# wangjie212/ManiSDP-matlab

Measured on AMD Instinct MI355X. Metric: tCG Hess-vec prods/sec (n,p), G81 MaxCut, higher is better.
Workload: dtype f64; 1 GPU; Gset G81 MaxCut, ManiSDP_onlyunitdiag RTR call, n=20000, p=32; n=20000, p=32, nnz_C=92644, TR_maxiter=40, TR_maxinner=100, parallelism=rows1

## Files before the change

manisdp-matlab_amd/csrc/msdp_pipe.h:

```cpp
#pragma once
#include <type_traits>
#include "msdp_psync.h"

template <class F>
__device__ __forceinline__ bool psync8(unsigned long long* slots, unsigned gen, int G, double (&v)[8], double* sh8, double* shb8, int* err,
                                       int bid, int backoff, unsigned long long* tr, F on_ready) {
    const int lane = threadIdx.x & 63, w = threadIdx.x >> 6;
    {
        const bool h8 = (lane & 8) != 0;
        double a[4], b[2], x;
#pragma unroll
        for (int k = 0; k < 4; ++k) a[k] = msdp_swap_add<32>(v[k], v[4 + k]);
#pragma unroll
        for (int k = 0; k < 2; ++k) b[k] = msdp_swap_add<16>(a[k], a[2 + k]);
        x = (h8 ? b[1] : b[0]) + msdp_dpp<0x128>(h8 ? b[0] : b[1]);
        x += msdp_dpp<MSDP_DPP_XOR1>(x); x += msdp_dpp<MSDP_DPP_XOR2>(x); x += msdp_dpp<MSDP_DPP_HALF_MIRROR>(x);
        if ((lane & 7) == 0) sh8[(lane >> 3) * PWAVES + w] = x;
    }
    if (tr && threadIdx.x == 0) tr[4] = __builtin_readcyclecounter();
    asm volatile("s_waitcnt vmcnt(0)" ::: "memory");
    __syncthreads();
    if (tr && threadIdx.x == 0) tr[2] = __builtin_readcyclecounter();
    {
        unsigned long long* gbase = slots + (size_t)(gen % PSYNC_GEN) * PSYNC_REP * PSYNC_NV * MSDP_MAX_GRID;
        if (w == 0) {
            const int rep = lane / PSYNC_NV, vi = lane % PSYNC_NV;
            double s = 0.0;
            for (int i = 0; i < PWAVES; ++i) s += sh8[vi * PWAVES + i];
            asm volatile("s_waitcnt vmcnt(0)" ::: "memory");
            __hip_atomic_store(gbase + ((size_t)rep * PSYNC_NV + vi) * MSDP_MAX_GRID + bid,
                               (unsigned long long)__double_as_longlong(s), __ATOMIC_RELAXED, __HIP_MEMORY_SCOPE_AGENT);
        }
        const unsigned long long* p0 = gbase + ((size_t)(bid & (PSYNC_REP - 1)) * PSYNC_NV + w) * MSDP_MAX_GRID + lane;
        double r0;
        int spins = 0;
        bool fail = false;
        const int first = ((backoff >> 16) & 0xff) ? ((backoff >> 16) & 0xff) : 27;
        for (int q = 0; q < first; ++q) __builtin_amdgcn_s_sleep(1);
        if (tr && threadIdx.x == 0) tr[3] = __builtin_readcyclecounter();
        for (;;) {
            unsigned long long b0[4];
            asm volatile(
                "global_load_dwordx2 %0, %4, off sc1\n\t"
                "global_load_dwordx2 %1, %4, off offset:512 sc1\n\t"
                "global_load_dwordx2 %2, %4, off offset:1024 sc1\n\t"
                "global_load_dwordx2 %3, %4, off offset:1536 sc1\n\t"
                "s_waitcnt vmcnt(0)"
                : "=&v"(b0[0]), "=&v"(b0[1]), "=&v"(b0[2]), "=&v"(b0[3])
                : "v"(p0)
                : "memory");
            bool ok = true;
            double t0 = 0.0;
#pragma unroll
            for (int q = 0; q < 4; ++q) {
                if (lane + 64 * q < G) {
                    ok = ok && b0[q] != PSYNC_SENT;
                    t0 += __longlong_as_double((long long)b0[q]);
                }
            }
            r0 = t0;
            if (__builtin_amdgcn_ballot_w64(!ok) == 0ULL) break;
            ++spins;
            if (spins > PSYNC_SPIN_LIMIT ||
                ((spins & 1023) == 0 && __hip_atomic_load(err, __ATOMIC_RELAXED, __HIP_MEMORY_SCOPE_AGENT))) { fail = true; break; }
            for (int q = 0; q < ((backoff >> 8) & 0xff); ++q) __builtin_amdgcn_s_sleep(1);
        }
        if (tr && threadIdx.x == 0) tr[7] = (__builtin_readcyclecounter() << 4) + (unsigned long long)(spins < 15 ? spins : 15);
        if (!fail) on_ready();
        r0 = msdp_wave_sum(r0);
        if (lane == 0) {
            shb8[w] = r0; shb8[8 + w] = fail ? 1.0 : 0.0;
            if (fail) __hip_atomic_store(err, 1, __ATOMIC_RELAXED, __HIP_MEMORY_SCOPE_AGENT);
        }
        if (w == 0)
            __hip_atomic_store(slots + (size_t)((gen + PSYNC_GEN - 1) % PSYNC_GEN) * PSYNC_REP * PSYNC_NV * MSDP_MAX_GRID +
                                   (size_t)lane * MSDP_MAX_GRID + bid,
                               PSYNC_SENT, __ATOMIC_RELAXED, __HIP_MEMORY_SCOPE_AGENT);
    }
    asm volatile("s_waitcnt lgkmcnt(0)\n\ts_barrier" ::: "memory");
    double bad = 0.0;
#pragma unroll
    for (int i = 0; i < 8; ++i) { v[i] = msdp_readlane(shb8[i], 0); bad += msdp_readlane(shb8[8 + i], 0); }
    return bad == 0.0;
}

typedef unsigned long long v2ul __attribute__((ext_vector_type(2)));
template <class F>
__device__ __forceinline__ bool psync8_lines(unsigned long long* slots, unsigned gen, int G, double (&v)[8], double* sh8, double* shp, double* shb8,
                                             int* err, int bid, int backoff, unsigned long long* tr, F on_ready) {
    const int lane = threadIdx.x & 63, w = threadIdx.x >> 6;
    {
        const bool h8 = (lane & 8) != 0;
        double a[4], b[2], x;
#pragma unroll
        for (int k = 0; k < 4; ++k) a[k] = msdp_swap_add<32>(v[k], v[4 + k]);
#pragma unroll
        for (int k = 0; k < 2; ++k) b[k] = msdp_swap_add<16>(a[k], a[2 + k]);
        x = (h8 ? b[1] : b[0]) + msdp_dpp_all<0x128>(h8 ? b[0] : b[1]);
        x += msdp_dpp_all<MSDP_DPP_XOR1>(x); x += msdp_dpp_all<MSDP_DPP_XOR2>(x); x += msdp_dpp_all<MSDP_DPP_HALF_MIRROR>(x);
        if ((lane & 7) == 0) sh8[(lane >> 3) * PWAVES + w] = x;
    }
    if (tr && threadIdx.x == 0) tr[4] = __builtin_readcyclecounter();
    asm volatile("s_waitcnt vmcnt(0)" ::: "memory");
    __syncthreads();
    if (tr && threadIdx.x == 0) tr[2] = __builtin_readcyclecounter();
    unsigned long long* gbase = slots + (size_t)(gen % PSYNC_GEN) * PSYNC_REP * PSYNC_NV * MSDP_MAX_GRID;
    if (w == 0) {
        const int rep = lane >> 3, vi = lane & 7;
        double s = 0.0;
        for (int i = 0; i < PWAVES; ++i) s += sh8[vi * PWAVES + i];
        asm volatile("s_waitcnt vmcnt(0)" ::: "memory");
        __hip_atomic_store(gbase + (size_t)rep * PSYNC_NV * MSDP_MAX_GRID + (size_t)bid * 8 + vi,
                           (unsigned long long)__double_as_longlong(s), __ATOMIC_RELAXED, __HIP_MEMORY_SCOPE_AGENT);
    }
    const unsigned long long* p0 = gbase + (size_t)(bid & (PSYNC_REP - 1)) * PSYNC_NV * MSDP_MAX_GRID + (size_t)(32 * w + (lane >> 2)) * 8 + 2 * (lane & 3);
    const bool in0 = 32 * w + (lane >> 2) < G, in1 = 32 * w + 16 + (lane >> 2) < G;
    double t0 = 0.0, t1 = 0.0;
    int spins = 0;
    bool fail = false;
    const int first = ((backoff >> 16) & 0xff) ? ((backoff >> 16) & 0xff) : (backoff & 0xff);
    for (int q = 0; q < first; ++q) __builtin_amdgcn_s_sleep(1);
    if (tr && threadIdx.x == 0) tr[3] = __builtin_readcyclecounter();
    if (__builtin_amdgcn_ballot_w64(in0) != 0ULL) {
        for (;;) {
            v2ul a0, a1;
            asm volatile(
                "global_load_dwordx4 %0, %2, off sc1\n\t"
                "global_load_dwordx4 %1, %2, off offset:1024 sc1\n\t"
                "s_waitcnt vmcnt(0)"
                : "=&v"(a0), "=&v"(a1)
                : "v"(p0)
                : "memory");
            bool ok = true;
            t0 = 0.0; t1 = 0.0;
            if (in0) { ok = a0.x != PSYNC_SENT && a0.y != PSYNC_SENT; t0 = __longlong_as_double((long long)a0.x); t1 = __longlong_as_double((long long)a0.y); }
            if (in1) { ok = ok && a1.x != PSYNC_SENT && a1.y != PSYNC_SENT; t0 += __longlong_as_double((long long)a1.x); t1 += __longlong_as_double((long long)a1.y); }
            if (__builtin_amdgcn_ballot_w64(!ok) == 0ULL) break;
            ++spins;
            if (spins > PSYNC_SPIN_LIMIT ||
                ((spins & 1023) == 0 && __hip_atomic_load(err, __ATOMIC_RELAXED, __HIP_MEMORY_SCOPE_AGENT))) { fail = true; break; }
            for (int q = 0; q < ((backoff >> 8) & 0xff); ++q) __builtin_amdgcn_s_sleep(1);
        }
    }
    if (tr && threadIdx.x == 0) tr[7] = (__builtin_readcyclecounter() << 4) + (unsigned long long)(spins < 15 ? spins : 15);
    t0 += msdp_dpp_all<0x124>(t0); t1 += msdp_dpp_all<0x124>(t1);
    t0 += msdp_dpp_all<0x128>(t0); t1 += msdp_dpp_all<0x128>(t1);
    t0 = msdp_rowpair_sum<16>(t0); t1 = msdp_rowpair_sum<16>(t1);
    t0 = msdp_rowpair_sum<32>(t0); t1 = msdp_rowpair_sum<32>(t1);
    if (lane < 4) { shp[w * 8 + 2 * lane] = t0; shp[w * 8 + 2 * lane + 1] = t1; }
    if (lane == 0) {
        shb8[8 + w] = fail ? 1.0 : 0.0;
        if (fail) __hip_atomic_store(err, 1, __ATOMIC_RELAXED, __HIP_MEMORY_SCOPE_AGENT);
    }
    asm volatile("s_waitcnt lgkmcnt(0)\n\ts_barrier" ::: "memory");
    on_ready();
    if (w == 0)
        __hip_atomic_store(slots + (size_t)((gen + PSYNC_GEN - 1) % PSYNC_GEN) * PSYNC_REP * PSYNC_NV * MSDP_MAX_GRID +
                               (size_t)(lane >> 3) * PSYNC_NV * MSDP_MAX_GRID + (size_t)bid * 8 + (lane & 7),
                           PSYNC_SENT, __ATOMIC_RELAXED, __HIP_MEMORY_SCOPE_AGENT);
    double s = 0.0;
#pragma unroll
    for (int k = 0; k < PWAVES; ++k) s += shp[k * 8 + (lane & 7)];
    const double fl = shb8[8 + (lane & 7)];
#pragma unroll
    for (int i = 0; i < 8; ++i) v[i] = msdp_readlane(s, i);
    return __builtin_amdgcn_ballot_w64(fl != 0.0) == 0ULL;
}

__device__ __forceinline__ bool pbar8_lines(unsigned long long* slots, unsigned gen, int G, double* shb8, int* err, int bid, int backoff) {
    const int lane = threadIdx.x & 63, w = threadIdx.x >> 6;
    asm volatile("s_waitcnt vmcnt(0)" ::: "memory");
    __syncthreads();
    unsigned long long* gbase = slots + (size_t)(gen % PSYNC_GEN) * PSYNC_REP * PSYNC_NV * MSDP_MAX_GRID;
    if (w == 0) {
        asm volatile("s_waitcnt vmcnt(0)" ::: "memory");
        __hip_atomic_store(gbase + (size_t)(lane >> 3) * PSYNC_NV * MSDP_MAX_GRID + (size_t)bid * 8 + (lane & 7), 0ULL, __ATOMIC_RELAXED, __HIP_MEMORY_SCOPE_AGENT);
    }
    const unsigned long long* p0 = gbase + (size_t)(bid & (PSYNC_REP - 1)) * PSYNC_NV * MSDP_MAX_GRID + (size_t)(32 * w + (lane >> 2)) * 8 + 2 * (lane & 3);
    const bool in0 = 32 * w + (lane >> 2) < G, in1 = 32 * w + 16 + (lane >> 2) < G;
    int spins = 0;
    bool fail = false;
    const int first = ((backoff >> 16) & 0xff) ? ((backoff >> 16) & 0xff) : (backoff & 0xff);
    for (int q = 0; q < first; ++q) __builtin_amdgcn_s_sleep(1);
    if (__builtin_amdgcn_ballot_w64(in0) != 0ULL) {
        for (;;) {
            v2ul a0, a1;
            asm volatile(
                "global_load_dwordx4 %0, %2, off sc1\n\t"
                "global_load_dwordx4 %1, %2, off offset:1024 sc1\n\t"
                "s_waitcnt vmcnt(0)"
                : "=&v"(a0), "=&v"(a1)
                : "v"(p0)
                : "memory");
            bool ok = true;
            if (in0) ok = a0.x != PSYNC_SENT && a0.y != PSYNC_SENT;
            if (in1) ok = ok && a1.x != PSYNC_SENT && a1.y != PSYNC_SENT;
            if (__builtin_amdgcn_ballot_w64(!ok) == 0ULL) break;
            ++spins;
            if (spins > PSYNC_SPIN_LIMIT ||
                ((spins & 1023) == 0 && __hip_atomic_load(err, __ATOMIC_RELAXED, __HIP_MEMORY_SCOPE_AGENT))) { fail = true; break; }
            for (int q = 0; q < ((backoff >> 8) & 0xff); ++q) __builtin_amdgcn_s_sleep(1);
        }
    }
    if (lane == 0) {
        shb8[8 + w] = fail ? 1.0 : 0.0;
        if (fail) __hip_atomic_store(err, 1, __ATOMIC_RELAXED, __HIP_MEMORY_SCOPE_AGENT);
    }
    asm volatile("s_waitcnt lgkmcnt(0)\n\ts_barrier" ::: "memory");
    if (w == 0)
        __hip_atomic_store(slots + (size_t)((gen + PSYNC_GEN - 1) % PSYNC_GEN) * PSYNC_REP * PSYNC_NV * MSDP_MAX_GRID +
                               (size_t)(lane >> 3) * PSYNC_NV * MSDP_MAX_GRID + (size_t)bid * 8 + (lane & 7),
                           PSYNC_SENT, __ATOMIC_RELAXED, __HIP_MEMORY_SCOPE_AGENT);
    const double fl = shb8[8 + (lane & 7)];
    return __builtin_amdgcn_ballot_w64(fl != 0.0) == 0ULL;
}

template <class F>
__device__ __forceinline__ bool psync2_8(unsigned long long* blk, unsigned long long* const* peers, int N, int me, int ri, unsigned gen, int G,
                                         double (&v)[8], double* sh8, double* shb8, int* err, int bid, int backoff, F on_ready) {
    const int lane = threadIdx.x & 63, w = threadIdx.x >> 6;
    {
        const bool h8 = (lane & 8) != 0;
        double a[4], b[2], x;
#pragma unroll
        for (int k = 0; k < 4; ++k) a[k] = msdp_swap_add<32>(v[k], v[4 + k]);
#pragma unroll
        for (int k = 0; k < 2; ++k) b[k] = msdp_swap_add<16>(a[k], a[2 + k]);
        x = (h8 ? b[1] : b[0]) + msdp_dpp<0x128>(h8 ? b[0] : b[1]);
        x += msdp_dpp<MSDP_DPP_XOR1>(x); x += msdp_dpp<MSDP_DPP_XOR2>(x); x += msdp_dpp<MSDP_DPP_HALF_MIRROR>(x);
        if ((lane & 7) == 0) sh8[(lane >> 3) * PWAVES + w] = x;
    }
    asm volatile("s_waitcnt vmcnt(0)" ::: "memory");
    __syncthreads();
    unsigned long long* ls = blk + (size_t)ri * XR2_REGION;
    unsigned long long* ml = ls + PSYNC_REGION;
    unsigned long long* gbase = ls + (size_t)(gen % PSYNC_GEN) * PSYNC_REP * PSYNC_NV * MSDP_MAX_GRID;
    if (w == 0 && lane < 8) {
        double s = 0.0;
        for (int i = 0; i < PWAVES; ++i) s += sh8[lane * PWAVES + i];
        asm volatile("s_waitcnt vmcnt(0)" ::: "memory");
        __hip_atomic_store(gbase + (size_t)lane * MSDP_MAX_GRID + bid, (unsigned long long)__double_as_longlong(s), __ATOMIC_RELAXED, __HIP_MEMORY_SCOPE_AGENT);
    }
    bool fail = false;
    if (bid == 0) {
        const unsigned long long* p0 = gbase + (size_t)w * MSDP_MAX_GRID + lane;
        double r0 = 0.0;
        int spins = 0;
        for (;;) {
            unsigned long long b0[4];
            asm volatile(
                "global_load_dwordx2 %0, %4, off sc1\n\t"
                "global_load_dwordx2 %1, %4, off offset:512 sc1\n\t"
                "global_load_dwordx2 %2, %4, off offset:1024 sc1\n\t"
                "global_load_dwordx2 %3, %4, off offset:1536 sc1\n\t"
                "s_waitcnt vmcnt(0)"
                : "=&v"(b0[0]), "=&v"(b0[1]), "=&v"(b0[2]), "=&v"(b0[3])
                : "v"(p0)
                : "memory");
            bool ok = true;
            double t0 = 0.0;
#pragma unroll
            for (int q = 0; q < 4; ++q) {
                if (lane + 64 * q < G) {
                    ok = ok && b0[q] != PSYNC_SENT;
                    t0 += __longlong_as_double((long long)b0[q]);
                }
            }
            r0 = t0;
            if (__builtin_amdgcn_ballot_w64(!ok) == 0ULL) break;
            ++spins;
            if (spins > PSYNC_SPIN_LIMIT || ((spins & 1023) == 0 && __hip_atomic_load(err, __ATOMIC_RELAXED, __HIP_MEMORY_SCOPE_AGENT))) { fail = true; break; }
        }
        r0 = msdp_wave_sum(r0);
        if (!fail && lane < N)
            __hip_atomic_store(peers[lane] + (size_t)ri * XR2_REGION + PSYNC_REGION + ((size_t)(gen % PSYNC_GEN) * 8 + me) * 8 + w,
                               (unsigned long long)__double_as_longlong(r0), __ATOMIC_RELAXED, __HIP_MEMORY_SCOPE_SYSTEM);
        if (fail) xr2_fail(blk, peers, N, err);
        if (w > 0 && lane == 0) shb8[8 + w] = fail ? 1.0 : 0.0;
    }
    if (w == 0) {
        const unsigned long long* p = ml + (size_t)(gen % PSYNC_GEN) * 64 + lane;
        const bool need = (lane >> 3) < N;
        const int first = bid == 0 ? 0 : (((backoff >> 16) & 0xff) ? ((backoff >> 16) & 0xff) : (backoff & 0xff));
        for (int q = 0; q < first; ++q) __builtin_amdgcn_s_sleep(1);
        unsigned long long x = 0ULL;
        int spins = 0;
        for (;;) {
            x = ld_u64_sys(p);
            if (__builtin_amdgcn_ballot_w64(need && x == PSYNC_SENT) == 0ULL) break;
            ++spins;
            if (spins > PSYNC_SPIN_LIMIT || ((spins & 1023) == 0 && __hip_atomic_load(err, __ATOMIC_RELAXED, __HIP_MEMORY_SCOPE_AGENT))) { fail = true; break; }
            for (int q = 0; q < ((backoff >> 8) & 0xff); ++q) __builtin_amdgcn_s_sleep(1);
        }
        double t = need ? __longlong_as_double((long long)x) : 0.0;
        t += msdp_dpp<0x128>(t);
        t = msdp_rowpair_sum<16>(t);
        t = msdp_rowpair_sum<32>(t);
        if (lane < 8) { shb8[lane] = t; if (bid != 0 && lane > 0) shb8[8 + lane] = 0.0; }
        if (lane == 0) shb8[8] = fail ? 1.0 : 0.0;
        if (fail) xr2_fail(blk, peers, N, err);
        if (lane < PSYNC_NV)
            __hip_atomic_store(ls + (size_t)((gen + PSYNC_GEN - 1) % PSYNC_GEN) * PSYNC_REP * PSYNC_NV * MSDP_MAX_GRID + (size_t)lane * MSDP_MAX_GRID + bid,
                               PSYNC_SENT, __ATOMIC_RELAXED, __HIP_MEMORY_SCOPE_AGENT);
        if (bid == 0)
            __hip_atomic_store(ml + (size_t)((gen + PSYNC_GEN - 1) % PSYNC_GEN) * 64 + lane, PSYNC_SENT, __ATOMIC_RELAXED, __HIP_MEMORY_SCOPE_AGENT);
    }
    __syncthreads();
    on_ready();
    double bad = 0.0;
#pragma unroll
    for (int i = 0; i < 8; ++i) { v[i] = msdp_readlane(shb8[i], 0); bad += msdp_readlane(shb8[8 + i], 0); }
    return bad == 0.0;
}

#ifndef MSDP_PIPE_LINES
#define MSDP_PIPE_LINES 1
#endif
#if MSDP_PIPE_LINES
#define PSYNC8(slots, gen, G, v, sh8, shb8, err, bid, backoff, tr, f) psync8_lines(slots, gen, G, v, sh8, shp, shb8, err, bid, backoff, tr, f)
#else
#define PSYNC8(slots, gen, G, v, sh8, shb8, err, bid, backoff, tr, f) psync8(slots, gen, G, v, sh8, shb8, err, bid, backoff, tr, f)
#endif
template <int LPR, int EW, int R, bool TRACE, bool FUSE, int XRM = 0, int EP = 1>
__device__ __forceinline__ void tcg_pipe_body(const Dev& d, unsigned long long* slots, int* err, const int bx) {
    constexpr bool XR = XRM != 0, XTWO = XRM == 2;
    constexpr bool CSR = EW == 0;
    static_assert(!XR || (!FUSE && !TRACE), "cross-rank instances: per-iteration launches");
    static_assert(R <= 5, "pipelined trip: every vector in registers");
    static_assert(CSR ? (EP == 64 / LPR && !XR && !TRACE) : EP == 1, "CSR rows: one row per wave, one rank");
    static_assert(PSYNC_NV == 8 && PSYNC_REP * PSYNC_NV == 64, "psync8 posts one slot per lane of wave 0");
    constexpr bool BSTORE = XRM == 0 && EW == 5 && !(FUSE && LPR == 8);
    constexpr bool BOFF = !(EW == 8 && LPR == 16), ROWB_INV = !XTWO;
    extern __shared__ double lds[];
    __shared__ double sh8[8 * PWAVES];
    __shared__ double shp[8 * PWAVES];
    __shared__ double shb8[16];
    constexpr int RPW = 64 / (LPR * EP);
    constexpr int RSTEP = PWAVES * RPW;
    constexpr int ROWS = R * RSTEP;
    double2* Ys = reinterpret_cast<double2*>(lds);
    double2* Gs = Ys + R * PB;
    double* eGs = reinterpret_cast<double*>(Gs + R * PB);
    double* vs = eGs + ROWS;
    int* cs = reinterpret_cast<int*>(vs + EW * ROWS);
    int* ls = cs + EW * ROWS;
    double2* HQs = reinterpret_cast<double2*>(ls + EW * ROWS);
    unsigned long long* pds = reinterpret_cast<unsigned long long*>(HQs + 2 * R * PB);
    double2* YPs = HQs + 2 * R * PB;
    double2* GPs = YPs + R * PB;
    double* EGPs = reinterpret_cast<double*>(GPs + R * PB);

    const Ctl* c = d.ctl;
    const bool lead = bx == 0 && threadIdx.x == 0;
    const int k_tr = c->k;
    if (c->done) {
        if (lead) {
            frame_store(&d.F[0], c->gg, c->gg, 0.0, 0.0, 0.0, sqrt(c->gg), 0.0, 0.0, 0, 0, 5, 0, 0, 1);
            d.ctl->tcg_running = 0;
            msdp_publish(d, k_tr, 0, 0);
        }
        return;
    }
    if (lead && !FUSE) msdp_publish(d, k_tr, 0, 1);
    const int bid = (XR && !XTWO) ? d.xr_gid0 + bx : bx;
    const int GS = (XR && !XTWO) ? d.xr_gtot : d.G;
    const int xri = k_tr & 1;
    __shared__ unsigned long long* shpeer[XTWO ? 8 : 1];
    if (XTWO) {
        if (threadIdx.x < 8) shpeer[threadIdx.x] = threadIdx.x < d.xr2_n ? d.xr2_peers[threadIdx.x] : d.xr2_blk;
        psync2_reset_other(d.xr2_blk, xri ^ 1, bid, GS);
        asm volatile("s_waitcnt vmcnt(0)" ::: "memory");
    } else if (XR) {
        unsigned long long* other = slots + (size_t)(xri ^ 1) * PSYNC_REGION;
        slots += (size_t)xri * PSYNC_REGION;
        psync_reset_other(other, bid, GS);
        asm volatile("s_waitcnt vmcnt(0)" ::: "memory");
    } else if (!FUSE) psync_reset_other(slots + PSYNC_REGION, bid, GS);
    int lo, hi;
    msdp_chunk_rows(d.n_loc, d.G, lo, hi, 0, bx);
    const int lane = threadIdx.x & 63, wave = threadIdx.x >> 6;
    const int sub = lane & (LPR - 1), rsub = lane / (LPR * EP);
    const int epi = (lane / LPR) & (EP - 1);
    const bool colok_g = 2 * sub < d.ld;
    const bool colok = colok_g && epi == 0;
    int cur = c->cur;
    const bool bench = c->bench_mode != 0;
    double Delta = c->Delta;
    const double kappa = c->kappa, theta = c->theta;
    const int mininner = c->mininner, maxinner = c->maxinner;
    double gg = c->gg;
    double fx = c->fx;
    int k_it = c->k;
    const double Delta_bar = c->Delta_bar, rho_prime = c->rho_prime, rho_reg_opt = c->rho_reg, tolgradnorm = c->tolgradnorm;
    const int maxiter = c->maxiter;
    int n_acc = c->accepted, n_rej = c->rejected, n_hv = c->hessvecs, n_ce = c->cost_evals;
    const double* __restrict__ Yl = cur ? d.Y[1] : d.Y[0];
    const double* __restrict__ gl = cur ? d.Gr[1] : d.Gr[0];
    const double* __restrict__ eGl = cur ? d.eG[1] : d.eG[0];
    const int slot0 = wave * RPW + rsub;
#define SLOT(r) ((r) * RSTEP + slot0)
#define ROW(r) (lo + SLOT(r))
#define ROK(r) (ROW(r) < hi)
#define OK(r) (ROK(r) && colok)
    const unsigned rowb0 = ((unsigned)(lo + slot0) * (unsigned)d.ld + 2u * (unsigned)sub) * 8u;
#define ROWB(r) (ROWB_INV ? (rowb0 + (unsigned)((r) * RSTEP) * (unsigned)d.ld * 8u) : (((unsigned)ROW(r) * gld + 2 * sub) * 8u))
    const int refresh = c->pipe_refresh;
    const int backoff = (c->psync_backoff & 0xff00ffff) | ((((c->psync_backoff >> 16) & 0xff) ? ((c->psync_backoff >> 16) & 0xff) : (c->psync8_backoff & 0xff)) << 16);
    const double2 zz = make_double2(0.0, 0.0);
    const unsigned gld = (unsigned)d.ld;
    constexpr bool LOC = !CSR && R * EW <= 15;
    constexpr bool MULTI = LOC && !(FUSE && LPR >= 16);
    double2 eta[R], rr[R], md[R], hmd[R], cmd[R], ctr[R];
#pragma unroll
    for (int r = 0; r < R; ++r) {
        const bool rok = ROK(r);
        const int rc = rok ? ROW(r) : lo;
        const int64_t o = (int64_t)rc * d.ld + (colok ? 2 * sub : 0);
        double2 y = ld2(Yl + o), g = ld2(gl + o);
        if (!OK(r)) { y = zz; g = zz; }
        Ys[r * PB + threadIdx.x] = y; Gs[r * PB + threadIdx.x] = g;
        eta[r] = zz; rr[r] = g; md[r] = g; hmd[r] = zz; cmd[r] = zz; ctr[r] = zz;
    }
#pragma unroll 1
    for (int r = 0; r < (CSR ? 0 : R); ++r) {
        const bool rok = ROK(r);
        const int rc = rok ? ROW(r) : lo;
        const double egv = eGl[rc];
        int cw[EW > 0 ? EW : 1];
        double vw[EW > 0 ? EW : 1];
#pragma unroll
        for (int w = 0; w < EW; ++w) {
            cw[w] = XR ? d.xr_ellc[(int64_t)w * d.ell_stride + rc] : d.ellc[(int64_t)w * d.ell_stride + rc];
            vw[w] = d.ellv[(int64_t)w * d.ell_stride + rc];
        }
        int kw[EW > 0 ? EW : 1];
#pragma unroll
        for (int w = 0; w < EW; ++w) {
            if (!rok) vw[w] = 0.0;
            kw[w] = vw[w] == 0.0 ? 3 : (cw[w] == rc ? 0 : ((cw[w] >= lo && cw[w] < hi) ? 1 : 2));
        }
#pragma unroll
        for (int a = 0; a < (LOC ? EW - 1 : 0); ++a)
#pragma unroll
            for (int b2 = 0; b2 < EW - 1 - a; ++b2)
                if (kw[b2] > kw[b2 + 1]) {
                    const int tk = kw[b2]; kw[b2] = kw[b2 + 1]; kw[b2 + 1] = tk;
                    const int tc = cw[b2]; cw[b2] = cw[b2 + 1]; cw[b2 + 1] = tc;
                    const double tv = vw[b2]; vw[b2] = vw[b2 + 1]; vw[b2 + 1] = tv;
                }
        if (XR && sub == 0) {
#pragma unroll
            for (int t = 0; t < 2; ++t)
                pds[t * ROWS + SLOT(r)] = rok ? d.xr_paddr[(int64_t)t * d.n_loc + rc] : 0ULL;
        }
        if (sub == 0) {
            eGs[SLOT(r)] = rok ? egv : 0.0;
#pragma unroll
            for (int w = 0; w < EW; ++w) {
                cs[w * ROWS + SLOT(r)] = BOFF ? (int)((unsigned)cw[w] * gld * 8u) : cw[w];
                vs[w * ROWS + SLOT(r)] = vw[w];
                const int li = cw[w] - lo;
                const int el = (li / RSTEP) * PB + (li % RSTEP) * LPR;
                ls[w * ROWS + SLOT(r)] = kw[w] == 2 ? -1 : (kw[w] == 3 ? (2 << 24) : ((kw[w] == 0 ? (1 << 24) : 0) | el));
            }
        }
    }
    if (CSR) {
#pragma unroll
        for (int r = 0; r < R; ++r)
            if (sub == 0 && epi == 0) eGs[SLOT(r)] = ROK(r) ? eGl[ROW(r)] : 0.0;
    }
    __syncthreads();
    int nl = 0;
    if (LOC && c->pipe_local != 0) {
        bool lead_ok = true;
#pragma unroll
        for (int w = 0; w < EW; ++w) {
            bool glob = false;
#pragma unroll
            for (int r = 0; r < R; ++r) glob = glob || ls[w * ROWS + SLOT(r)] < 0;
            lead_ok = lead_ok && __builtin_amdgcn_ballot_w64(glob) == 0ULL;
            if (lead_ok) nl = w + 1;
        }
    }
    unsigned gen = 0;
    const unsigned half_bytes = XR ? (unsigned)(((size_t)d.xr_cap + (size_t)d.xr_halo) * d.ld * sizeof(double)) : (unsigned)((size_t)d.n_loc * d.ld * sizeof(double));
    const __amdgpu_buffer_rsrc_t rs_md = XR ? __builtin_amdgcn_make_buffer_rsrc(d.xr_rows[0], 0, 4u * half_bytes, 0x00020000)
                                            : __builtin_amdgcn_make_buffer_rsrc(d.mdx, 0, (FUSE ? 7u : 4u) * half_bytes, 0x00020000);
    const unsigned st_records = (unsigned)hi * (unsigned)d.ld * 8u;
    const unsigned rowbs = rowb0 | (colok ? 0u : 0x80000000u);
    auto row_store = [&](unsigned reg, int r, double2 val) {
        st2_sc1(__builtin_amdgcn_make_buffer_rsrc(reinterpret_cast<char*>(d.mdx) + (size_t)reg * half_bytes, 0, st_records, 0x00020000),
                rowbs + (unsigned)(r * RSTEP) * (unsigned)d.ld * 8u, val);
    };
    bool xr_has_push = false, xr_has_push2 = false;
    if (XR) {
        bool any = false, any2 = false;
#pragma unroll
        for (int r = 0; r < R; ++r) { any = any || pds[SLOT(r)] != 0ULL; any2 = any2 || pds[ROWS + SLOT(r)] != 0ULL; }
        xr_has_push2 = __builtin_amdgcn_ballot_w64(any2) != 0ULL;
        xr_has_push = xr_has_push2 || __builtin_amdgcn_ballot_w64(any) != 0ULL;
    }
    auto xr_push = [&](int r, unsigned reg, double2 val) {
        if (!XR || !xr_has_push) return;
#pragma unroll
        for (int t = 0; t < 2; ++t) {
            if (t == 1 && !xr_has_push2) continue;
            const unsigned long long a = pds[t * ROWS + SLOT(r)];
            if (a != 0ULL && OK(r)) {
                double* ptr = reinterpret_cast<double*>(a + (unsigned long long)reg * half_bytes) + 2 * sub;
                if (XTWO) {
                    __hip_atomic_store(ptr, val.x, __ATOMIC_RELAXED, __HIP_MEMORY_SCOPE_SYSTEM);
                    __hip_atomic_store(ptr + 1, val.y, __ATOMIC_RELAXED, __HIP_MEMORY_SCOPE_SYSTEM);
                } else {
                    __hip_atomic_store(ptr, val.x, __ATOMIC_RELAXED, __HIP_MEMORY_SCOPE_AGENT);
                    __hip_atomic_store(ptr + 1, val.y, __ATOMIC_RELAXED, __HIP_MEMORY_SCOPE_AGENT);
                }
            }
        }
    };
    __amdgpu_buffer_rsrc_t rs_g = __builtin_amdgcn_make_buffer_rsrc(cur ? d.Gr[1] : d.Gr[0], 0, half_bytes, 0x00020000);
    unsigned g_base = 0u;
    const unsigned gcol = colok ? 2 * sub : 0, gcol8 = gcol * 8u;
    const bool idle_lanes = d.ld < 2 * LPR;
    constexpr int CSR_CB = 8;
    constexpr bool CSR_KEEP = CSR && R <= 2 && !FUSE;
    int ckeep[CSR_KEEP ? R : 1][CSR_CB];
    double vkeep[CSR_KEEP ? R : 1][CSR_CB];
    if (CSR_KEEP) {
#pragma unroll
        for (int r = 0; r < R; ++r) {
            const bool rok = ROK(r);
            const int s0 = rok ? d.rowptr[ROW(r)] : 0, s1 = rok ? d.rowptr[ROW(r) + 1] : 0;
#pragma unroll
            for (int u = 0; u < CSR_CB; ++u) {
                const int k = s0 + epi + u * EP;
                const bool in = k < s1;
                ckeep[r][u] = in ? d.colind[k] : (rok ? ROW(r) : lo);
                vkeep[r][u] = in ? d.cval[k] : 0.0;
            }
        }
    }
    auto csr_gather = [&](int r, __amdgpu_buffer_rsrc_t rs, unsigned base) -> double2 {
        constexpr int CB = CSR_CB;
        double2 acc = make_double2(0.0, 0.0);
        const bool rok = ROK(r);
        const int s0 = (CSR && rok) ? d.rowptr[ROW(r)] : 0, s1 = (CSR && rok) ? d.rowptr[ROW(r) + 1] : 0;
        const unsigned gcg = colok_g ? 2 * sub : 0;
        int kfirst = s0 + epi;
        if (CSR_KEEP) {
            double2 x[CB];
#pragma unroll
            for (int u = 0; u < CB; ++u) x[u] = ld2_sc1(rs, base + ((unsigned)ckeep[CSR_KEEP ? r : 0][u] * gld + gcg) * 8u);
#pragma unroll
            for (int u = 0; u < CB; ++u) { const double cv = vkeep[CSR_KEEP ? r : 0][u]; acc.x = fma(cv, x[u].x, acc.x); acc.y = fma(cv, x[u].y, acc.y); }
            kfirst += CB * EP;
        }
        for (int k0 = kfirst; __builtin_amdgcn_ballot_w64(k0 < s1) != 0ULL; k0 += CB * EP) {
            double2 x[CB];
            double cvk[CB];
#pragma unroll
            for (int u = 0; u < CB; ++u) {
                const int k = k0 + u * EP;
                const bool in = k < s1;
                const int cidx = in ? d.colind[k] : (rok ? ROW(r) : lo);
                cvk[u] = in ? d.cval[k] : 0.0;
                x[u] = ld2_sc1(rs, base + ((unsigned)cidx * gld + gcg) * 8u);
            }
#pragma unroll
            for (int u = 0; u < CB; ++u) { acc.x = fma(cvk[u], x[u].x, acc.x); acc.y = fma(cvk[u], x[u].y, acc.y); }
        }
#pragma unroll
        for (int m = LPR; m < LPR * EP; m <<= 1) { acc.x += __shfl_xor(acc.x, m); acc.y += __shfl_xor(acc.y, m); }
        if (!colok) acc = make_double2(0.0, 0.0);
        return acc;
    };

    double z_r = gg, d_Pd = gg, e_Pd = 0.0, e_Pe = 0.0, model_value = 0.0, alpha = 0.0, beta = 0.0;
    double norm_r0 = sqrt(gg);
    int j = 0, stop = 5;
    int pub_cd = refresh > 0 ? refresh : 0;
    const int k_it0 = c->k;
#define FSTAMP(ph) do { if (TRACE && FUSE && threadIdx.x == 0 && k_it - k_it0 < MSDP_TRACE_NJ) \
        d.trace[((size_t)bx * MSDP_TRACE_NJ + (k_it - k_it0)) * 8 + (ph)] = __builtin_readcyclecounter(); } while (0)
    bool first = true, direct = false, failed = false;
    unsigned xq = 0;
    bool have_x = false;
#define MSDP_TRACE_KSEL 7
#define FTRIP_ON (TRACE && FUSE && k_it - k_it0 == MSDP_TRACE_KSEL && j < MSDP_TRACE_NJ)
#define FTRIP_PTR (d.trace + (size_t)GS * MSDP_TRACE_NJ * 8 + ((size_t)bx * MSDP_TRACE_NJ + j) * 8)
#define PTSTAMP(ph) do { if (!FUSE) { TSTAMP(ph); } else if (FTRIP_ON && threadIdx.x == 0) FTRIP_PTR[ph] = __builtin_readcyclecounter(); } while (0)
  auto trips = [&](auto nlc) {
    constexpr int NL = decltype(nlc)::value;
    constexpr int NG = EW - NL;
#ifndef MSDP_PIPE_VARIANT
#define MSDP_PIPE_VARIANT 0
#endif
    constexpr bool PREF = !CSR && R * NG <= ((FUSE && MSDP_PIPE_VARIANT == 0) ? 9 : 15);
    constexpr bool SPLIT = (MSDP_PIPE_VARIANT == 2 && FUSE) ? true : !PREF;
    double2 X[R][NG > 0 ? NG : 1];
    for (;;) {
        PTSTAMP(0);
#define PIPE_ISSUE(rs, base, w0) do { \
            _Pragma("unroll") for (int r = 0; r < R; ++r) \
            _Pragma("unroll") for (int w = 0; w < NG; ++w) { \
                if ((w0) + w < EW) { \
                    const unsigned coff = (unsigned)cs[((w0) + w) * ROWS + SLOT(r)]; \
                    X[r][w] = ld2_cp<XTWO ? 17 : MSDP_CPOL_SC1>((rs), (base) + (BOFF ? coff + gcol8 : (coff * gld + gcol) * 8u)); } } } while (0)
#define PIPE_FOLDX(r, acc, w0) do { \
            _Pragma("unroll") for (int w = 0; w < NG; ++w) { \
                if ((w0) + w < EW) { \
                    const double vv = vs[((w0) + w) * ROWS + SLOT(r)]; \
                    (acc).x = fma(vv, X[r][w].x, (acc).x); (acc).y = fma(vv, X[r][w].y, (acc).y); } } } while (0)
#define PIPE_FOLDL(r, acc, src) do { \
            _Pragma("unroll") for (int w = 0; w < NL; ++w) { \
                const double vv = vs[w * ROWS + SLOT(r)]; \
                const double2 xx = (src)[(ls[w * ROWS + SLOT(r)] & 0xffffff) + sub]; \
                (acc).x = fma(vv, xx.x, (acc).x); (acc).y = fma(vv, xx.y, (acc).y); } } while (0)
#define PIPE_GATHER_ALL(rs, base, dst) do { \
            if (CSR) { _Pragma("unroll") for (int r = 0; r < R; ++r) (dst)[r] = csr_gather(r, (rs), (base)); break; } \
            _Pragma("unroll") for (int r = 0; r < R; ++r) (dst)[r] = zz; \
            _Pragma("unroll") for (int w0 = 0; w0 < EW; w0 += (NG > 0 ? NG : 1)) { \
                PIPE_ISSUE(rs, base, w0); \
                _Pragma("unroll") for (int r = 0; r < R; ++r) PIPE_FOLDX(r, (dst)[r], w0); } \
            if (!colok) { _Pragma("unroll") for (int r = 0; r < R; ++r) (dst)[r] = zz; } } while (0)
        double v[8] = {0.0, 0.0, 0.0, 0.0, 0.0, 0.0, 0.0, 0.0};
        auto pre_sums = [&]() {
            if (!SPLIT) return;
#pragma unroll
            for (int r = 0; r < R; ++r) {
                const double2 g = Gs[r * PB + threadIdx.x], mdr = md[r], e0 = eta[r], rv = rr[r];
                const double2 rg = make_double2(rv.x - g.x, rv.y - g.y);
                v[3] += mdr.x * g.x + mdr.y * g.y;
                v[5] += mdr.x * rg.x + mdr.y * rg.y;
                v[6] += rv.x * rv.x + rv.y * rv.y;
                v[7] += (e0.x * g.x + e0.y * g.y) + 0.5 * (e0.x * rg.x + e0.y * rg.y);
            }
        };
        if (first) {
            pre_sums();
            PIPE_GATHER_ALL(rs_g, g_base, cmd);
#pragma unroll
            for (int r = 0; r < R; ++r) ctr[r] = cmd[r];
        } else {
            if (direct) {
                PIPE_GATHER_ALL(rs_md, 3u * half_bytes, ctr);
                PIPE_GATHER_ALL(rs_md, 2u * half_bytes, cmd);
            }
            if (!CSR && !have_x) PIPE_ISSUE(rs_md, (xq ^ 1u) * half_bytes, NL);
            pre_sums();
            auto products = [&](auto masked) {
#pragma unroll
                for (int r = 0; r < R; ++r) {
                    double2 a = zz;
                    if (CSR) a = csr_gather(r, rs_md, (xq ^ 1u) * half_bytes);
                    else { PIPE_FOLDL(r, a, HQs + (xq ^ 1u) * R * PB); PIPE_FOLDX(r, a, NL); }
                    if (decltype(masked)::value && !colok) a = zz;
                    ctr[r].x = fma(-alpha, a.x, ctr[r].x); ctr[r].y = fma(-alpha, a.y, ctr[r].y);
                    cmd[r].x = fma(beta, cmd[r].x, ctr[r].x); cmd[r].y = fma(beta, cmd[r].y, ctr[r].y);
                }
            };
            if (!CSR && idle_lanes) products(std::true_type()); else products(std::false_type());
        }
        have_x = false;
        bool pub = --pub_cd == 0;
        if (pub) pub_cd = refresh;
        pub = pub && !first;
#pragma unroll
        for (int r = 0; r < R; ++r) {
            const double2 acc = cmd[r];
            const double2 y = Ys[r * PB + threadIdx.x], mdr = md[r], rv = rr[r];
            const double dot = msdp_group_sum_all<LPR>(acc.x * y.x + acc.y * y.y);
            const double eg = eGs[SLOT(r)];
            const double2 hq = make_double2(acc.x - y.x * dot - mdr.x * eg, acc.y - y.y * dot - mdr.y * eg);
            hmd[r] = hq;
            if (MULTI) HQs[xq * R * PB + r * PB + threadIdx.x] = hq;
            if (BSTORE) row_store(xq, r, hq);
            else if (OK(r)) st2_sc1(rs_md, xq * half_bytes + ROWB(r), hq);
            xr_push(r, xq, hq);
            if (!SPLIT) {
                const double2 g = Gs[r * PB + threadIdx.x], e0 = eta[r];
                const double2 rg = make_double2(rv.x - g.x, rv.y - g.y);
                v[0] += mdr.x * hq.x + mdr.y * hq.y;
                v[1] += rv.x * hq.x + rv.y * hq.y;
                v[2] += hq.x * hq.x + hq.y * hq.y;
                v[3] += mdr.x * g.x + mdr.y * g.y;
                v[4] += e0.x * hq.x + e0.y * hq.y;
                v[5] += mdr.x * rg.x + mdr.y * rg.y;
                v[6] += rv.x * rv.x + rv.y * rv.y;
                v[7] += (e0.x * g.x + e0.y * g.y) + 0.5 * (e0.x * rg.x + e0.y * rg.y);
            }
        }
        if (pub) {
#pragma unroll
            for (int r = 0; r < R; ++r) {
                const double2 y = Ys[r * PB + threadIdx.x], mdr = md[r], rv = rr[r];
                const double dn = msdp_group_sum_all<LPR>(rv.x * y.x + rv.y * y.y);
                if (BSTORE) {
                    row_store(2u, r, mdr);
                    row_store(3u, r, make_double2(rv.x - y.x * dn, rv.y - y.y * dn));
                } else if (OK(r)) {
                    st2_sc1(rs_md, 2u * half_bytes + ROWB(r), mdr);
                    st2_sc1(rs_md, 3u * half_bytes + ROWB(r), make_double2(rv.x - y.x * dn, rv.y - y.y * dn));
                }
                xr_push(r, 2u, mdr);
                xr_push(r, 3u, make_double2(rv.x - y.x * dn, rv.y - y.y * dn));
            }
        }
        if (SPLIT) {
#pragma unroll
            for (int r = 0; r < R; ++r) {
                const double2 hq = hmd[r], mdr = md[r], e0 = eta[r], rv = rr[r];
                v[0] += mdr.x * hq.x + mdr.y * hq.y;
                v[1] += rv.x * hq.x + rv.y * hq.y;
                v[2] += hq.x * hq.x + hq.y * hq.y;
                v[4] += e0.x * hq.x + e0.y * hq.y;
            }
        }
        PTSTAMP(1);
        if (TRACE && FUSE && j == 0) { FSTAMP(1); }
        auto next_gather = [&]() { if (PREF && !pub) { PIPE_ISSUE(rs_md, xq * half_bytes, NL); have_x = true; } };
        if (XTWO) {
            if (!psync2_8(d.xr2_blk, shpeer, d.xr2_n, d.xr2_me, xri, gen++, GS + d.xr2_skip, v, sh8, shb8, err, bid, backoff, next_gather)) { failed = true; break; }
        } else
        if (!PSYNC8(slots, gen++, GS, v, sh8, shb8, err, bid, backoff,
                    (TRACE && !FUSE && j >= MSDP_TRACE_J0 && j < MSDP_TRACE_J0 + MSDP_TRACE_NJ) ? d.trace + ((size_t)bx * MSDP_TRACE_NJ + (j - MSDP_TRACE_J0)) * 8 :
                    (FTRIP_ON ? FTRIP_PTR : nullptr),
                    next_gather)) { failed = true; break; }
        PTSTAMP(5);
        const double d_Hd = v[0];
        z_r = v[6];
        model_value = v[7];
        alpha = z_r / d_Hd;
        const double e_Pe_new = e_Pe + 2.0 * alpha * e_Pd + alpha * alpha * d_Pd;
        if (!bench && (d_Hd <= 0.0 || e_Pe_new >= Delta * Delta)) {
            const double tau = (-e_Pd + sqrt(e_Pd * e_Pd + d_Pd * (Delta * Delta - e_Pe))) / d_Pd;
#pragma unroll
            for (int r = 0; r < R; ++r) {
                eta[r].x -= tau * md[r].x; eta[r].y -= tau * md[r].y;
                rr[r].x -= tau * hmd[r].x; rr[r].y -= tau * hmd[r].y;
            }
            stop = (d_Hd <= 0.0) ? 1 : 2;
            ++j;
            break;
        }
        const double new_model = model_value - alpha * v[3] - 0.5 * alpha * (v[4] + v[5]) + 0.5 * alpha * alpha * d_Hd;
        const double r_r = fmax(z_r - 2.0 * alpha * v[1] + alpha * alpha * v[2], 0.0);
        e_Pe = e_Pe_new;
        if (!bench && new_model >= model_value) { stop = 6; ++j; break; }
#pragma unroll
        for (int r = 0; r < R; ++r) {
            eta[r].x -= alpha * md[r].x; eta[r].y -= alpha * md[r].y;
            rr[r].x -= alpha * hmd[r].x; rr[r].y -= alpha * hmd[r].y;
        }
        model_value = new_model;
        ++j;
        const double norm_r = sqrt(r_r);
        const double nr0t = (theta == 1.0) ? norm_r0 : pow(norm_r0, theta);
        if (!bench && j >= mininner && norm_r <= norm_r0 * fmin(nr0t, kappa)) {
            stop = (kappa < nr0t) ? 3 : 4;
            break;
        }
        if (j >= maxinner) break;
        beta = r_r / z_r;
        e_Pd = beta * (e_Pd + alpha * d_Pd);
        d_Pd = r_r + beta * beta * d_Pd;
        z_r = r_r;
#pragma unroll
        for (int r = 0; r < R; ++r) {
            const double2 y = Ys[r * PB + threadIdx.x];
            const double2 vv = make_double2(rr[r].x + beta * md[r].x, rr[r].y + beta * md[r].y);
            const double dot = msdp_group_sum_all<LPR>(vv.x * y.x + vv.y * y.y);
            md[r] = make_double2(vv.x - y.x * dot, vv.y - y.y * dot);
        }
        direct = pub;
        first = false;
        xq ^= 1u;
        { --j; PTSTAMP(6); ++j; }
    }
#undef PIPE_ISSUE
#undef PIPE_FOLDX
#undef PIPE_FOLDL
#undef PIPE_GATHER_ALL
#undef PTSTAMP
#undef FTRIP_ON
#undef FTRIP_PTR
  };
  if (XR && !XTWO && d.xr2_skip && bid == 0) return;
  if (XR) {
#pragma unroll
    for (int r = 0; r < R; ++r) {
        if (OK(r)) st2_sc1(rs_md, 2u * half_bytes + ROWB(r), md[r]);
        xr_push(r, 2u, md[r]);
    }
    asm volatile("s_waitcnt vmcnt(0)" ::: "memory");
    if (XTWO) {
        double z0 = 0.0, z1 = 0.0, z2 = 0.0;
        if (!psync2(d.xr2_blk, shpeer, d.xr2_n, d.xr2_me, xri, gen++, GS + d.xr2_skip, 0, z0, z1, z2, sh8, shb8, err, bid, backoff, false)) return;
    } else if (!pbar8_lines(slots, gen++, GS, shb8, err, bid, backoff)) return;
    rs_g = rs_md; g_base = 2u * half_bytes;
  }
  bool first_tr = true;
  for (;;) {
    FSTAMP(0);
    if (FUSE && !first_tr) {
#pragma unroll
        for (int r = 0; r < R; ++r) {
            const double2 g = Gs[r * PB + threadIdx.x];
            eta[r] = zz; rr[r] = g; md[r] = g; hmd[r] = zz; cmd[r] = zz; ctr[r] = zz;
        }
        z_r = gg; d_Pd = gg; e_Pd = 0.0; e_Pe = 0.0; model_value = 0.0; alpha = 0.0; beta = 0.0;
        norm_r0 = sqrt(gg);
        j = 0; stop = 5; first = true; direct = false; have_x = false;
        pub_cd = refresh > 0 ? refresh : 0;
    }
    first_tr = false;
    if (MULTI && nl >= 3) trips(std::integral_constant<int, MULTI ? 3 : 0>());
    else if (MULTI && nl == 2) trips(std::integral_constant<int, MULTI ? 2 : 0>());
    else trips(std::integral_constant<int, 0>());
    if (failed) return;
    if (TRACE && FUSE && threadIdx.x == 0 && k_it - k_it0 < MSDP_TRACE_NJ)
        d.trace[((size_t)bx * MSDP_TRACE_NJ + (k_it - k_it0)) * 8 + 2] = (__builtin_readcyclecounter() & 0x00ffffffffffffffULL) | ((unsigned long long)(j & 0xff) << 56);
    if (!FUSE) {
#pragma unroll
        for (int r = 0; r < R; ++r) {
            if (OK(r)) {
                const int64_t o = (int64_t)ROW(r) * d.ld + 2 * sub;
                const double2 g = Gs[r * PB + threadIdx.x];
                st2(d.eta[0] + o, eta[r]);
                st2(d.Heta[0] + o, make_double2(rr[r].x - g.x, rr[r].y - g.y));
            }
        }
        if (lead) {
            frame_store(&d.F[0], z_r, d_Pd, e_Pd, e_Pe, model_value, norm_r0, alpha, beta, 0, j, stop, 0, 0, 0);
            d.ctl->tcg_running = 0;
            msdp_publish(d, k_tr, j, 0);
        }
        return;
    }
    double tv[8] = {0.0, 0.0, 0.0, 0.0, 0.0, 0.0, 0.0, 0.0};
    const unsigned yx_base = 4u * half_bytes, gx_base = (5u + (unsigned)(cur ^ 1)) * half_bytes;
#pragma unroll
    for (int r = 0; r < R; ++r) {
        const double2 y = Ys[r * PB + threadIdx.x], g = Gs[r * PB + threadIdx.x];
        const double2 e0 = eta[r];
        const double2 he = make_double2(rr[r].x - g.x, rr[r].y - g.y);
        tv[2] += e0.x * (g.x + 0.5 * he.x) + e0.y * (g.y + 0.5 * he.y);
        const double2 x = make_double2(y.x + e0.x, y.y + e0.y);
        const double nn = sqrt(fmax(msdp_group_sum_all<LPR>(x.x * x.x + x.y * x.y), 2.2250738585072014e-308));
        const double2 ypr = make_double2(x.x / nn, x.y / nn);
        YPs[r * PB + threadIdx.x] = ypr;
        if (BSTORE) row_store(4u, r, ypr);
        else if (OK(r)) st2_sc1(rs_md, yx_base + ROWB(r), ypr);
    }
    FSTAMP(3);
    if (!pbar8_lines(slots, gen++, GS, shb8, err, bid, backoff)) return;
    FSTAMP(4);
    auto prop_finish = [&](int r, double2 acc) {
        if (!colok) acc = zz;
        const double2 ypr = YPs[r * PB + threadIdx.x];
        const double dot = msdp_group_sum_all<LPR>(acc.x * ypr.x + acc.y * ypr.y);
        const double2 gpr = make_double2(acc.x - ypr.x * dot, acc.y - ypr.y * dot);
        GPs[r * PB + threadIdx.x] = gpr;
        tv[1] += gpr.x * gpr.x + gpr.y * gpr.y;
        if (sub == 0 && epi == 0) {
            EGPs[SLOT(r)] = dot;
            tv[0] += 0.5 * dot;
        }
        if (BSTORE) row_store(5u + (unsigned)(cur ^ 1), r, gpr);
        else if (OK(r)) st2_sc1(rs_md, gx_base + ROWB(r), gpr);
    };
    if (CSR) {
#pragma unroll
        for (int r = 0; r < R; ++r) prop_finish(r, csr_gather(r, rs_md, yx_base));
    } else if (R * EW <= 16) {
        double2 XG[R][EW > 0 ? EW : 1];
#pragma unroll
        for (int r = 0; r < R; ++r)
#pragma unroll
            for (int w = 0; w < EW; ++w) XG[r][w] = ld2_sc1(rs_md, yx_base + (BOFF ? (unsigned)cs[w * ROWS + SLOT(r)] + gcol8 : ((unsigned)cs[w * ROWS + SLOT(r)] * gld + gcol) * 8u));
#pragma unroll
        for (int r = 0; r < R; ++r) {
            double2 acc = zz;
#pragma unroll
            for (int w = 0; w < EW; ++w) { const double vv = vs[w * ROWS + SLOT(r)]; acc.x = fma(vv, XG[r][w].x, acc.x); acc.y = fma(vv, XG[r][w].y, acc.y); }
            prop_finish(r, acc);
        }
    } else {
#pragma unroll 1
        for (int r = 0; r < R; ++r) {
            double2 xw[EW > 0 ? EW : 1];
#pragma unroll
            for (int w = 0; w < EW; ++w) xw[w] = ld2_sc1(rs_md, yx_base + (BOFF ? (unsigned)cs[w * ROWS + SLOT(r)] + gcol8 : ((unsigned)cs[w * ROWS + SLOT(r)] * gld + gcol) * 8u));
            double2 acc = zz;
#pragma unroll
            for (int w = 0; w < EW; ++w) { const double vv = vs[w * ROWS + SLOT(r)]; acc.x = fma(vv, xw[w].x, acc.x); acc.y = fma(vv, xw[w].y, acc.y); }
            prop_finish(r, acc);
        }
    }
    FSTAMP(5);
    if (!PSYNC8(slots, gen++, GS, tv, sh8, shb8, err, bid, backoff, nullptr, []() {})) return;
    FSTAMP(6);
    {
        const double fp = tv[0], ggp = tv[1], prd = tv[2];
        double rhonum = fx - fp;
        double rhoden = -prd;
        const double rreg = fmax(1.0, fabs(fx)) * 2.220446049250313e-16 * rho_reg_opt;
        rhonum += rreg;
        rhoden += rreg;
        const bool model_decreased = rhoden >= 0.0;
        const double rho = rhonum / rhoden;
        if (rho < 0.25 || !model_decreased || isnan(rho)) Delta = Delta / 4.0;
        else if (rho > 0.75 && (stop == 1 || stop == 2)) Delta = fmin(2.0 * Delta, Delta_bar);
        const bool accept = model_decreased && rho > rho_prime;
        if (accept) ++n_acc; else ++n_rej;
        n_hv += j;
        ++n_ce;
        if (lead) {
            Ctl* cw = d.ctl;
            cw->rho = rho; cw->rhonum = rhonum; cw->rhoden = rhoden; cw->fx_prop = fp; cw->gg_prop = ggp;
            cw->accepted = n_acc; cw->rejected = n_rej; cw->hessvecs = n_hv; cw->cost_evals = n_ce;
            cw->last_stop_inner = stop;
        }
        if (accept) {
            cur ^= 1;
            fx = fp; gg = ggp;
            { double2* t = Ys; Ys = YPs; YPs = t; }
            { double2* t = Gs; Gs = GPs; GPs = t; }
            { double* t = eGs; eGs = EGPs; EGPs = t; }
            rs_g = rs_md; g_base = gx_base;
        }
        FSTAMP(7);
        ++k_it;
    }
    if (sqrt(gg) < tolgradnorm || k_it >= maxiter) break;
  }
    {
        double* Yo = cur ? d.Y[1] : d.Y[0];
        double* Go = cur ? d.Gr[1] : d.Gr[0];
        double* eo = cur ? d.eG[1] : d.eG[0];
#pragma unroll
        for (int r = 0; r < R; ++r) {
            if (OK(r)) {
                const int64_t o = (int64_t)ROW(r) * d.ld + 2 * sub;
                st2(Yo + o, Ys[r * PB + threadIdx.x]);
                st2(Go + o, Gs[r * PB + threadIdx.x]);
            }
            if (sub == 0 && ROK(r)) eo[ROW(r)] = eGs[SLOT(r)];
        }
    }
    if (lead) {
        Ctl* cw = d.ctl;
        cw->fx = fx; cw->gg = gg; cw->norm_grad = sqrt(gg); cw->Delta = Delta;
        cw->k = k_it; cw->cur = cur;
        cw->done = 1;
        cw->tcg_running = 0;
        frame_store(&d.F[0], 0.0, 0.0, 0.0, 0.0, 0.0, 0.0, 0.0, 0.0, 0, 0, stop, 0, 0, 0);
    }
#undef FSTAMP
#undef SLOT
#undef ROW
#undef ROK
#undef OK
#undef ROWB
}

template <int LPR, int EW, int R, bool TRACE = false, bool FUSE = false, int XRM = 0, int EP = 1>
__global__ __launch_bounds__(PB) void k_tcg_pipe_obl(Dev d, unsigned long long* slots, int* err) {
    tcg_pipe_body<LPR, EW, R, TRACE, FUSE, XRM, EP>(d, slots, err, (int)blockIdx.x);
}
```

Baseline: 210,200 Hess-vec/s.

## Spread next-gather loads across CG update and park recurrences in LDS

For the fused LPR=16, EW=5, R=3 instance, the gather loads for the next Hessian-vector product are no longer issued in one burst inside the barrier callback. They are split into five chunks interleaved with the scalar CG update, the eta/r updates and the md projection, so the loads overlap with that arithmetic. The ctr/cmd recurrences are parked in LDS (reusing HQs) to relieve register pressure, and pow(norm_r0, theta) is hoisted out of the inner loop. The MSDP_PIPE_VARIANT switch is removed. This risks more LDS traffic and scheduling changes, and it depends on HQs being unused in this instance.

```diff
diff --git a/manisdp-matlab_amd/csrc/msdp_pipe.h b/manisdp-matlab_amd/csrc/msdp_pipe.h
--- a/manisdp-matlab_amd/csrc/msdp_pipe.h
+++ b/manisdp-matlab_amd/csrc/msdp_pipe.h
@@ -410,6 +410,10 @@
     const unsigned gld = (unsigned)d.ld;
     constexpr bool LOC = !CSR && R * EW <= 15;
     constexpr bool MULTI = LOC && !(FUSE && LPR >= 16);
+    constexpr bool PARK = FUSE && LPR == 16 && EW == 5 && R == 3;
+    static_assert(!PARK || !MULTI, "the parked recurrences live in HQs: the instance must not keep its rows of H md there");
+    double2* CTs = HQs;
+    double2* CMs = HQs + R * PB;
     double2 eta[R], rr[R], md[R], hmd[R], cmd[R], ctr[R];
 #pragma unroll
     for (int r = 0; r < R; ++r) {
@@ -578,6 +582,7 @@
 
     double z_r = gg, d_Pd = gg, e_Pd = 0.0, e_Pe = 0.0, model_value = 0.0, alpha = 0.0, beta = 0.0;
     double norm_r0 = sqrt(gg);
+    double nr0t_tcg = norm_r0;
     int j = 0, stop = 5;
     int pub_cd = refresh > 0 ? refresh : 0;
     const int k_it0 = c->k;
@@ -593,11 +598,15 @@
   auto trips = [&](auto nlc) {
     constexpr int NL = decltype(nlc)::value;
     constexpr int NG = EW - NL;
-#ifndef MSDP_PIPE_VARIANT
-#define MSDP_PIPE_VARIANT 0
-#endif
-    constexpr bool PREF = !CSR && R * NG <= ((FUSE && MSDP_PIPE_VARIANT == 0) ? 9 : 15);
-    constexpr bool SPLIT = (MSDP_PIPE_VARIANT == 2 && FUSE) ? true : !PREF;
+    constexpr bool PREF = !CSR && R * NG <= (FUSE ? 9 : 15);
+    constexpr bool SPREAD = PARK;
+    constexpr bool SPLIT = !PREF;
+    constexpr int NGD = NG > 0 ? NG : 1;
+#define PIPE_ISSUE_PART(base, ka, kb) do { \
+            _Pragma("unroll") for (int k = (ka); k < (kb); ++k) { \
+                const unsigned coff = (unsigned)cs[(NL + k % NGD) * ROWS + SLOT(k / NGD)]; \
+                X[k / NGD][k % NGD] = ld2_cp<XTWO ? 17 : MSDP_CPOL_SC1>(rs_md, (base) + (BOFF ? coff + gcol8 : (coff * gld + gcol) * 8u)); } } while (0)
+#define PIPE_SPREAD(ka, kb) do { if (SPREAD && !pub) PIPE_ISSUE_PART(xq * half_bytes, ka, kb); } while (0)
     double2 X[R][NG > 0 ? NG : 1];
     for (;;) {
         PTSTAMP(0);
@@ -649,6 +658,10 @@
             }
             if (!CSR && !have_x) PIPE_ISSUE(rs_md, (xq ^ 1u) * half_bytes, NL);
             pre_sums();
+            if (PARK && !direct) {
+#pragma unroll
+                for (int r = 0; r < R; ++r) { ctr[r] = CTs[r * PB + threadIdx.x]; cmd[r] = CMs[r * PB + threadIdx.x]; }
+            }
             auto products = [&](auto masked) {
 #pragma unroll
                 for (int r = 0; r < R; ++r) {
@@ -669,6 +682,7 @@
 #pragma unroll
         for (int r = 0; r < R; ++r) {
             const double2 acc = cmd[r];
+            if (PARK) { CTs[r * PB + threadIdx.x] = ctr[r]; CMs[r * PB + threadIdx.x] = acc; }
             const double2 y = Ys[r * PB + threadIdx.x], mdr = md[r], rv = rr[r];
             const double dot = msdp_group_sum_all<LPR>(acc.x * y.x + acc.y * y.y);
             const double eg = eGs[SLOT(r)];
@@ -719,7 +733,10 @@
         }
         PTSTAMP(1);
         if (TRACE && FUSE && j == 0) { FSTAMP(1); }
-        auto next_gather = [&]() { if (PREF && !pub) { PIPE_ISSUE(rs_md, xq * half_bytes, NL); have_x = true; } };
+        auto next_gather = [&]() {
+            if (SPREAD) { PIPE_SPREAD(0, 3); }
+            else if (PREF && !pub) { PIPE_ISSUE(rs_md, xq * half_bytes, NL); have_x = true; }
+        };
         if (XTWO) {
             if (!psync2_8(d.xr2_blk, shpeer, d.xr2_n, d.xr2_me, xri, gen++, GS + d.xr2_skip, v, sh8, shb8, err, bid, backoff, next_gather)) { failed = true; break; }
         } else
@@ -744,10 +761,12 @@
             ++j;
             break;
         }
+        PIPE_SPREAD(3, 6);
         const double new_model = model_value - alpha * v[3] - 0.5 * alpha * (v[4] + v[5]) + 0.5 * alpha * alpha * d_Hd;
         const double r_r = fmax(z_r - 2.0 * alpha * v[1] + alpha * alpha * v[2], 0.0);
         e_Pe = e_Pe_new;
         if (!bench && new_model >= model_value) { stop = 6; ++j; break; }
+        PIPE_SPREAD(6, 9);
 #pragma unroll
         for (int r = 0; r < R; ++r) {
             eta[r].x -= alpha * md[r].x; eta[r].y -= alpha * md[r].y;
@@ -756,7 +775,7 @@
         model_value = new_model;
         ++j;
         const double norm_r = sqrt(r_r);
-        const double nr0t = (theta == 1.0) ? norm_r0 : pow(norm_r0, theta);
+        const double nr0t = PARK ? nr0t_tcg : ((theta == 1.0) ? norm_r0 : pow(norm_r0, theta));
         if (!bench && j >= mininner && norm_r <= norm_r0 * fmin(nr0t, kappa)) {
             stop = (kappa < nr0t) ? 3 : 4;
             break;
@@ -766,6 +785,7 @@
         e_Pd = beta * (e_Pd + alpha * d_Pd);
         d_Pd = r_r + beta * beta * d_Pd;
         z_r = r_r;
+        PIPE_SPREAD(9, 12);
 #pragma unroll
         for (int r = 0; r < R; ++r) {
             const double2 y = Ys[r * PB + threadIdx.x];
@@ -773,12 +793,16 @@
             const double dot = msdp_group_sum_all<LPR>(vv.x * y.x + vv.y * y.y);
             md[r] = make_double2(vv.x - y.x * dot, vv.y - y.y * dot);
         }
+        PIPE_SPREAD(12, 15);
+        if (SPREAD) have_x = !pub;
         direct = pub;
         first = false;
         xq ^= 1u;
         { --j; PTSTAMP(6); ++j; }
     }
 #undef PIPE_ISSUE
+#undef PIPE_ISSUE_PART
+#undef PIPE_SPREAD
 #undef PIPE_FOLDX
 #undef PIPE_FOLDL
 #undef PIPE_GATHER_ALL
@@ -815,6 +839,8 @@
         pub_cd = refresh > 0 ? refresh : 0;
     }
     first_tr = false;
+    nr0t_tcg = norm_r0;
+    if (PARK && theta != 1.0) { asm volatile("" ::: "memory"); nr0t_tcg = pow(norm_r0, theta); }
     if (MULTI && nl >= 3) trips(std::integral_constant<int, MULTI ? 3 : 0>());
     else if (MULTI && nl == 2) trips(std::integral_constant<int, MULTI ? 2 : 0>());
     else trips(std::integral_constant<int, 0>());
```

After: 222,500 Hess-vec/s (median of 6 runs). 5.9% higher.
